# recmo/mpc-iris-code

Measured on AMD Instinct MI355X. Metric: template comparisons/sec (query×rotations×DB) + % HBM roofline, 1/2/4/8 GPU, higher is better.
Workload: dtype fp4 e2m1 MFMA -> f32 (0/+-1 products)

## Files before the change

mpc-iris-code_amd/csrc/iris_mfma.hip:

```cpp
#include <hip/hip_runtime.h>
#include <stdlib.h>

#include "iris_device.hpp"

namespace iris {

typedef int v8i __attribute__((ext_vector_type(8)));
typedef float v16f __attribute__((ext_vector_type(16)));

constexpr int kTileRecs = 32;
constexpr int kTileUint4 = kPlaneGroups * 64;
constexpr int kMfmaTiles = 4;
constexpr int kMfmaWgs = 2;
constexpr int kSplitStages = 6;
constexpr int kSplitT = 2;

__device__ __forceinline__ v16f mfma_fp4(const v8i &a, const v8i &b, const v16f &c) {
    return __builtin_amdgcn_mfma_scale_f32_32x32x64_f8f6f4(a, b, c, 4, 4, 0, 127, 0, 127);
}

struct QFrag {
    v8i am, ae;
};
__device__ __forceinline__ QFrag qfrag_of(const uint4 &qe) {
    QFrag f;
    f.ae = v8i{(int)qe.x, (int)qe.y, (int)qe.z, (int)qe.w, 0, 0, 0, 0};
    f.am = v8i{(int)(qe.x & 0x22222222u), (int)((qe.y & 0x22222222u) << 1), (int)(qe.z & 0x22222222u),
               (int)((qe.w & 0x22222222u) << 1), 0, 0, 0, 0};
    return f;
}

__device__ __forceinline__ void chunk_step(uint32_t x0, uint32_t x1, const QFrag &q, v16f &den, v16f &s) {
    const v8i bm = {(int)(x0 & 0x22222222u), (int)(x0 & 0x11111111u), (int)(x1 & 0x22222222u),
                    (int)(x1 & 0x11111111u), 0, 0, 0, 0};
    const v8i be = {(int)(x0 & 0xAAAAAAAAu), (int)((x0 << 1) & 0xAAAAAAAAu), (int)(x1 & 0xAAAAAAAAu),
                    (int)((x1 << 1) & 0xAAAAAAAAu), 0, 0, 0, 0};
    den = mfma_fp4(q.am, bm, den);
    s = mfma_fp4(q.ae, be, s);
}

typedef unsigned int u32x4 __attribute__((ext_vector_type(4)));
__device__ __forceinline__ uint4 stream_load(const uint4 *p) {
    const u32x4 v = __builtin_nontemporal_load((const u32x4 *)p);
    return make_uint4(v.x, v.y, v.z, v.w);
}

enum { MF_COUNTS = 0, MF_SEARCH = 1, MF_MATCH = 2, MF_TOPK = 3 };

template <int MODE, int T = kMfmaTiles, int KS = 1, bool FUSED = false>
__global__ void __launch_bounds__(64 * kWaveSlots, kMfmaWgs)
    template_mfma_kernel(const uint4 *__restrict__ db, const uint4 *__restrict__ qfrag, uint64_t tile0,
                         uint64_t ntiles, uint64_t first, uint64_t end, uint16_t *__restrict__ num_out,
                         uint16_t *__restrict__ den_out, double *__restrict__ dist_out,
                         Partial *__restrict__ partials, FusedFinish fin, MatchSink ms) {
    constexpr int W = kWaveSlots;
    static_assert(KS == 1 || (W % KS == 0 && kPlaneGroups % KS == 0), "K-split geometry");
    const int lane = threadIdx.x & 63;
    const int wslot = threadIdx.x >> 6;
    const int slice = wslot % KS;
    const uint64_t wave = (uint64_t)blockIdx.x * (W / KS) + wslot / KS;
    const uint64_t tw = wave * T;
    const bool active = tw < ntiles;
    constexpr int kG = kPlaneGroups / KS;
    const int g0 = slice * kG;

    v16f den[T], s[T];
#pragma unroll
    for (int t = 0; t < T; ++t) {
#pragma unroll
        for (int i = 0; i < 16; ++i) {
            den[t][i] = 0.f;
            s[t][i] = 0.f;
        }
    }

    if (active) {
        const uint4 *dp[T];
#pragma unroll
        for (int t = 0; t < T; ++t) {
            const uint64_t rel = (tw + t < ntiles) ? tw + t : ntiles - 1;
            dp[t] = db + (tile0 + rel) * (uint64_t)kTileUint4 + lane;
        }
        const uint4 *qp = qfrag + lane;
        struct Stage {
            uint4 d[T];
            uint4 q0, q1;
        };
        auto load = [&](Stage &st, int g) {
            g = (g < kG ? g : kG - 1) + g0;
#pragma unroll
            for (int t = 0; t < T; ++t) st.d[t] = stream_load(dp[t] + g * 64);
            st.q0 = qp[(2 * g) * 64];
            st.q1 = qp[(2 * g + 1) * 64];
            __builtin_amdgcn_sched_barrier(0);
        };
        auto compute = [&](const Stage &st) {
            const QFrag f0 = qfrag_of(st.q0);
#pragma unroll
            for (int t = 0; t < T; ++t) chunk_step(st.d[t].x, st.d[t].y, f0, den[t], s[t]);
            const QFrag f1 = qfrag_of(st.q1);
#pragma unroll
            for (int t = 0; t < T; ++t) chunk_step(st.d[t].z, st.d[t].w, f1, den[t], s[t]);
        };
        if constexpr (KS > 1) {
            Stage st[kSplitStages];
#pragma unroll
            for (int i = 0; i < kSplitStages - 1; ++i) load(st[i], i);
#pragma unroll
            for (int g = 0; g < kG; ++g) {
                if (g + kSplitStages - 1 < kG) load(st[(g + kSplitStages - 1) % kSplitStages], g + kSplitStages - 1);
                compute(st[g % kSplitStages]);
            }
        } else {
            Stage sa, sb, sc;
            load(sa, 0);
            load(sb, 1);
            int g = 0;
#pragma unroll 1
            for (; g + 3 <= kG; g += 3) {
                load(sc, g + 2);
                compute(sa);
                load(sa, g + 3);
                compute(sb);
                load(sb, g + 4);
                compute(sc);
            }
            if constexpr (kG % 3 >= 1) compute(sa);
            if constexpr (kG % 3 == 2) compute(sb);
        }
    }
    if constexpr (KS > 1) {
        __shared__ float red[W][T][32][64];
        if (slice != 0) {
#pragma unroll
            for (int t = 0; t < T; ++t)
#pragma unroll
                for (int i = 0; i < 16; ++i) {
                    red[wslot][t][i][lane] = den[t][i];
                    red[wslot][t][16 + i][lane] = s[t][i];
                }
        }
        __syncthreads();
        if (slice == 0) {
#pragma unroll
            for (int k = 1; k < KS; ++k)
#pragma unroll
                for (int t = 0; t < T; ++t)
#pragma unroll
                    for (int i = 0; i < 16; ++i) {
                        den[t][i] += red[wslot + k][t][i][lane];
                        s[t][i] += red[wslot + k][t][16 + i][lane];
                    }
        }
    }

    const int h = lane >> 5;
    Partial best = partial_none();
    bool hit[T];
    uint32_t hn[T], hd[T];
    int hr[T];
    uint64_t hi[T];
    uint64_t twe = tw, wave_e = wave;
    if constexpr (MODE == MF_TOPK) {
        uint32_t tx = threadIdx.x;
        asm volatile("" : "+v"(tx));
        wave_e = (uint64_t)blockIdx.x * (W / KS) + (tx >> 6) / KS;
        twe = wave_e * T;
    }
#pragma unroll
    for (int t = 0; t < T; ++t) {
        const uint64_t t0 = (tile0 + twe + t) * kTileRecs;
        const bool tv = active && (twe + t < ntiles) && slice == 0;
        if constexpr (MODE == MF_COUNTS) {
            __shared__ __attribute__((aligned(16))) uint16_t sh_out[W][1024];
            uint16_t *lds = sh_out[wslot];
            if (num_out)
                store_tile_rows(num_out, lds, t0, first, end, tv, lane,
                                [&](int r) { return (uint16_t)(((int)den[t][r] - (int)s[t][r]) >> 1); });
            if (den_out)
                store_tile_rows(den_out, lds, t0, first, end, tv, lane,
                                [&](int r) { return (uint16_t)(uint32_t)den[t][r]; });
        } else {
            const uint64_t tg = t0 + (lane & 31);
            const bool valid = tv && tg >= first && tg < end;
            const uint64_t o = tg - first;
            uint32_t bn, bd;
            int br;
            best_rotation(lane, [&](int r, uint32_t &nn, uint32_t &dd) {
                dd = (uint32_t)den[t][r];
                nn = (uint32_t)(((int)dd - (int)s[t][r]) >> 1);
            }, bn, bd, br);
            if constexpr (MODE == MF_MATCH) {
                hit[t] = match_hit(ms, valid && h == 0, bn, bd);
                hn[t] = bn;
                hd[t] = bd;
                hr[t] = br;
                hi[t] = o;
                continue;
            }
            if constexpr (MODE == MF_TOPK) {
                hn[t] = bn;
                hd[t] = valid && h == 0 ? bd : 0;
                hr[t] = br;
                continue;
            }
            if (valid && dist_out && h == 0) dist_out[o] = bd ? (double)bn / (double)bd : __builtin_inf();
            Partial c;
            c.num = bn;
            c.den = valid ? bd : 0;
            c.rot = br;
            c.pad = 0;
            c.idx = o;
            if (partial_better_dev(c, best)) best = c;
        }
    }
    if constexpr (MODE == MF_MATCH) append_matches<T>(ms, lane, hit, hn, hd, hr, hi);
    if constexpr (MODE == MF_TOPK) {
#pragma unroll
        for (int t = 0; t < T; ++t) {
            Partial c;
            c.num = hn[t];
            c.den = hd[t];
            c.rot = hr[t];
            c.pad = 0;
            c.idx = (tile0 + twe + t) * kTileRecs + (lane & 31) - first;
            topk_insert(best, (uint32_t)ms.cap, lane, c, true);
        }
        if (slice == 0) topk_store(ms, wave_e, lane, best);
    }
    if constexpr (MODE == MF_SEARCH) {
#pragma unroll
        for (int off = 32; off >= 1; off >>= 1) {
            const Partial ot = partial_shfl_xor(best, off);
            if (partial_better_dev(ot, best)) best = ot;
        }
        __shared__ Partial sh[W];
        if (lane == 0) sh[wslot] = best;
        __syncthreads();
        Partial b = sh[0];
        if (threadIdx.x == 0) {
#pragma unroll
            for (int w = 1; w < W; ++w)
                if (partial_better_dev(sh[w], b)) b = sh[w];
            if constexpr (!FUSED) partials[blockIdx.x] = b;
        }
        if constexpr (FUSED) fold_partials_last(partials, b, fin);
    }
}


struct QueryFrags {
    const uint4 *q[4];
};

template <int NQ>
__global__ void __launch_bounds__(256, 2)
    template_multi_kernel(const uint4 *__restrict__ db, QueryFrags qf, uint64_t tile0, uint64_t ntiles,
                          uint64_t first, uint64_t end, Partial *__restrict__ partials) {
    constexpr int T = 4 / NQ;
    const int lane = threadIdx.x & 63;
    const int wslot = threadIdx.x >> 6;
    const uint64_t wave = (uint64_t)blockIdx.x * kWaveSlots + wslot;
    const uint64_t tw = wave * T;
    const bool active = tw < ntiles;

    v16f den[NQ][T], s[NQ][T];
#pragma unroll
    for (int qi = 0; qi < NQ; ++qi)
#pragma unroll
        for (int t = 0; t < T; ++t)
#pragma unroll
            for (int i = 0; i < 16; ++i) {
                den[qi][t][i] = 0.f;
                s[qi][t][i] = 0.f;
            }

    if (active) {
        const uint4 *dp[T];
#pragma unroll
        for (int t = 0; t < T; ++t) {
            const uint64_t rel = (tw + t < ntiles) ? tw + t : ntiles - 1;
            dp[t] = db + (tile0 + rel) * (uint64_t)kTileUint4 + lane;
        }
        struct Stage {
            uint4 d[T];
            uint4 q[NQ][2];
        };
        auto load = [&](Stage &st, int g) {
            g = g < kPlaneGroups ? g : kPlaneGroups - 1;
#pragma unroll
            for (int t = 0; t < T; ++t) st.d[t] = stream_load(dp[t] + g * 64);
#pragma unroll
            for (int qi = 0; qi < NQ; ++qi) {
                st.q[qi][0] = qf.q[qi][(2 * g) * 64 + lane];
                st.q[qi][1] = qf.q[qi][(2 * g + 1) * 64 + lane];
            }
            __builtin_amdgcn_sched_barrier(0);
        };
        auto compute = [&](const Stage &st) {
#pragma unroll
            for (int qi = 0; qi < NQ; ++qi) {
                const QFrag f0 = qfrag_of(st.q[qi][0]);
#pragma unroll
                for (int t = 0; t < T; ++t) chunk_step(st.d[t].x, st.d[t].y, f0, den[qi][t], s[qi][t]);
                const QFrag f1 = qfrag_of(st.q[qi][1]);
#pragma unroll
                for (int t = 0; t < T; ++t) chunk_step(st.d[t].z, st.d[t].w, f1, den[qi][t], s[qi][t]);
            }
        };
        Stage sa, sb, sc;
        load(sa, 0);
        load(sb, 1);
        int g = 0;
#pragma unroll 1
        for (; g + 3 <= kPlaneGroups; g += 3) {
            load(sc, g + 2);
            compute(sa);
            load(sa, g + 3);
            compute(sb);
            load(sb, g + 4);
            compute(sc);
        }
        if (g < kPlaneGroups) compute(sa);
    }

    Partial best[NQ];
#pragma unroll
    for (int qi = 0; qi < NQ; ++qi) best[qi] = partial_none();
#pragma unroll
    for (int t = 0; t < T; ++t) {
        const uint64_t tg = (tile0 + tw + t) * kTileRecs + (lane & 31);
        const bool valid = active && (tw + t < ntiles) && tg >= first && tg < end;
#pragma unroll
        for (int qi = 0; qi < NQ; ++qi) {
            uint32_t bn, bd;
            int br;
            best_rotation(lane, [&](int r, uint32_t &nn, uint32_t &dd) {
                dd = (uint32_t)den[qi][t][r];
                nn = (uint32_t)(((int)dd - (int)s[qi][t][r]) >> 1);
            }, bn, bd, br);
            Partial c;
            c.num = bn;
            c.den = valid ? bd : 0;
            c.rot = br;
            c.pad = 0;
            c.idx = tg - first;
            if (partial_better_dev(c, best[qi])) best[qi] = c;
        }
    }
    __shared__ Partial sh[NQ][kWaveSlots];
#pragma unroll
    for (int qi = 0; qi < NQ; ++qi) {
#pragma unroll
        for (int off = 32; off >= 1; off >>= 1) {
            const Partial ot = partial_shfl_xor(best[qi], off);
            if (partial_better_dev(ot, best[qi])) best[qi] = ot;
        }
        if (lane == 0) sh[qi][wslot] = best[qi];
    }
    __syncthreads();
    if (threadIdx.x < NQ) {
        const int qi = threadIdx.x;
        Partial b = sh[qi][0];
#pragma unroll
        for (int w = 1; w < kWaveSlots; ++w)
            if (partial_better_dev(sh[qi][w], b)) b = sh[qi][w];
        partials[(uint64_t)qi * gridDim.x + blockIdx.x] = b;
    }
}


typedef const __attribute__((address_space(1))) u32x4 *GlobalFrag;
__device__ __forceinline__ uint4 frag_load(GlobalFrag p) {
    const u32x4 v = *p;
    return make_uint4(v.x, v.y, v.z, v.w);
}

template <int NQ, int T>
__device__ __forceinline__ void share_round(const uint4 *__restrict__ db, const GlobalFrag (&qf)[NQ], uint64_t tile0,
                                            uint64_t ntiles, uint64_t tw, uint64_t first, uint64_t end, int lane,
                                            Partial (&best)[NQ]) {
    const bool active = tw < ntiles;
    v16f den[NQ][T], s[NQ][T];
#pragma unroll
    for (int qi = 0; qi < NQ; ++qi)
#pragma unroll
        for (int t = 0; t < T; ++t)
#pragma unroll
            for (int i = 0; i < 16; ++i) {
                den[qi][t][i] = 0.f;
                s[qi][t][i] = 0.f;
            }

    if (active) {
        const uint4 *dp[T];
#pragma unroll
        for (int t = 0; t < T; ++t) {
            const uint64_t rel = (tw + t < ntiles) ? tw + t : ntiles - 1;
            dp[t] = db + (tile0 + rel) * (uint64_t)kTileUint4 + lane;
        }
        struct Stage {
            uint4 d[T];
            uint4 q[NQ][2];
        };
        auto load = [&](Stage &st, int g) {
            g = g < kPlaneGroups ? g : kPlaneGroups - 1;
#pragma unroll
            for (int t = 0; t < T; ++t) st.d[t] = stream_load(dp[t] + g * 64);
#pragma unroll
            for (int qi = 0; qi < NQ; ++qi) {
                st.q[qi][0] = frag_load(qf[qi] + (2 * g) * 64 + lane);
                st.q[qi][1] = frag_load(qf[qi] + (2 * g + 1) * 64 + lane);
            }
            __builtin_amdgcn_sched_barrier(0);
        };
        auto compute = [&](const Stage &st) {
#pragma unroll
            for (int qi = 0; qi < NQ; ++qi) {
                const QFrag f0 = qfrag_of(st.q[qi][0]);
#pragma unroll
                for (int t = 0; t < T; ++t) chunk_step(st.d[t].x, st.d[t].y, f0, den[qi][t], s[qi][t]);
                const QFrag f1 = qfrag_of(st.q[qi][1]);
#pragma unroll
                for (int t = 0; t < T; ++t) chunk_step(st.d[t].z, st.d[t].w, f1, den[qi][t], s[qi][t]);
            }
        };
        Stage sa, sb, sc;
        load(sa, 0);
        load(sb, 1);
        int g = 0;
#pragma unroll 1
        for (; g + 3 <= kPlaneGroups; g += 3) {
            load(sc, g + 2);
            compute(sa);
            load(sa, g + 3);
            compute(sb);
            load(sb, g + 4);
            compute(sc);
        }
        if constexpr (kPlaneGroups % 3 >= 1) compute(sa);
        if constexpr (kPlaneGroups % 3 == 2) compute(sb);
    }

#pragma unroll
    for (int t = 0; t < T; ++t) {
        const uint64_t tg = (tile0 + tw + t) * kTileRecs + (lane & 31);
        const bool valid = active && (tw + t < ntiles) && tg >= first && tg < end;
#pragma unroll
        for (int qi = 0; qi < NQ; ++qi) {
            uint32_t bn, bd;
            int br;
            best_rotation(lane, [&](int r, uint32_t &nn, uint32_t &dd) {
                dd = (uint32_t)den[qi][t][r];
                nn = (uint32_t)(((int)dd - (int)s[qi][t][r]) >> 1);
            }, bn, bd, br);
            Partial c;
            c.num = bn;
            c.den = valid ? bd : 0;
            c.rot = br;
            c.pad = 0;
            c.idx = tg - first;
            if (partial_better_dev(c, best[qi])) best[qi] = c;
        }
    }
}

template <int NQ, int N>
__device__ __forceinline__ void share_stash(Partial (&best)[NQ], int lane, int pos, Partial *sh) {
#pragma unroll
    for (int qi = 0; qi < NQ; ++qi) {
#pragma unroll
        for (int off = 32; off >= 1; off >>= 1) {
            const Partial ot = partial_shfl_xor(best[qi], off);
            if (partial_better_dev(ot, best[qi])) best[qi] = ot;
        }
        if (lane == 0) sh[qi * N + pos] = best[qi];
    }
}

typedef __attribute__((address_space(1))) Partial *GlobalPartial;
template <int NQ, int N>
__device__ __forceinline__ void share_finish(const Partial *sh, const GlobalPartial (&out)[NQ]) {
    __syncthreads();
    if (threadIdx.x < NQ) {
        const int qi = threadIdx.x;
        Partial b = sh[qi * N];
#pragma unroll
        for (int w = 1; w < N; ++w)
            if (partial_better_dev(sh[qi * N + w], b)) b = sh[qi * N + w];
        const GlobalPartial o = out[qi] + blockIdx.x;
        o->num = b.num;
        o->den = b.den;
        o->rot = b.rot;
        o->pad = b.pad;
        o->idx = b.idx;
    }
}

__global__ void __launch_bounds__(64 * kWaveSlots, kMfmaWgs)
    template_share_kernel(const uint4 *__restrict__ db, const uint4 *__restrict__ qfrag, uint64_t tile0, uint64_t ntiles,
                          uint64_t first, uint64_t end, Partial *__restrict__ partials, const GuestSlot *slot,
                          const uint32_t *own_done, unsigned long long *count, uint32_t even_only) {
    __shared__ uint32_t sh_flag[2];
    __shared__ uint64_t sh_guest[3];
    if (threadIdx.x == 0) {
        const uint32_t dn =
            own_done ? __hip_atomic_load(own_done + blockIdx.x, __ATOMIC_RELAXED, __HIP_MEMORY_SCOPE_AGENT) : 0u;
        uint32_t rdy = 0;
        if (slot && !dn && !(even_only && (blockIdx.x & 1)))
            rdy = __hip_atomic_load(&slot->ready, __ATOMIC_RELAXED, __HIP_MEMORY_SCOPE_AGENT);
        if (rdy) {
            __builtin_amdgcn_fence(__ATOMIC_ACQUIRE, "agent");
            sh_guest[0] = (uint64_t)slot->frag;
            sh_guest[1] = (uint64_t)slot->partials;
            sh_guest[2] = (uint64_t)slot->done;
        }
        sh_flag[0] = dn;
        sh_flag[1] = rdy;
    }
    __syncthreads();
    if (__builtin_amdgcn_readfirstlane(sh_flag[0])) return;
    const bool shared = __builtin_amdgcn_readfirstlane(sh_flag[1]) != 0;
    const int lane = threadIdx.x & 63;
    const int wslot = __builtin_amdgcn_readfirstlane(threadIdx.x >> 6);
    const uint64_t tw = ((uint64_t)blockIdx.x * kWaveSlots + wslot) * kMfmaTiles;
    auto uniform64 = [](uint64_t v) {
        const uint32_t lo = (uint32_t)__builtin_amdgcn_readfirstlane((int)(uint32_t)v);
        const uint32_t hi = (uint32_t)__builtin_amdgcn_readfirstlane((int)(uint32_t)(v >> 32));
        return (uint64_t)hi << 32 | lo;
    };
    constexpr int kRounds = kMfmaTiles / 2;
    __shared__ Partial sh_best[2 * kRounds * kWaveSlots];
    if (!shared) {
        Partial best[1] = {partial_none()};
        const GlobalFrag qf[1] = {(GlobalFrag)qfrag};
        share_round<1, kMfmaTiles>(db, qf, tile0, ntiles, tw, first, end, lane, best);
        share_stash<1, kWaveSlots>(best, lane, wslot, sh_best);
        const GlobalPartial out[1] = {(GlobalPartial)partials};
        share_finish<1, kWaveSlots>(sh_best, out);
        return;
    }
    const GlobalFrag qf[2] = {(GlobalFrag)qfrag, (GlobalFrag)uniform64(sh_guest[0])};
#pragma unroll
    for (int rd = 0; rd < kRounds; ++rd) {
        Partial best[2] = {partial_none(), partial_none()};
        share_round<2, 2>(db, qf, tile0, ntiles, tw + 2 * rd, first, end, lane, best);
        share_stash<2, kRounds * kWaveSlots>(best, lane, rd * kWaveSlots + wslot, sh_best);
    }
    const GlobalPartial out[2] = {(GlobalPartial)partials, (GlobalPartial)uniform64(sh_guest[1])};
    __attribute__((address_space(1))) uint32_t *const guest_done =
        (__attribute__((address_space(1))) uint32_t *)uniform64(sh_guest[2]);
    share_finish<2, kRounds * kWaveSlots>(sh_best, out);
    if (threadIdx.x == 1) {
        __hip_atomic_store(guest_done + blockIdx.x, 1u, __ATOMIC_RELAXED, __HIP_MEMORY_SCOPE_AGENT);
        if (count) atomicAdd(count, 1ull);
    }
}

__global__ void share_prepare_kernel(GuestSlot *slot, uint32_t *done, uint32_t n) {
    const uint32_t i = blockIdx.x * blockDim.x + threadIdx.x;
    if (i == 0) *slot = GuestSlot{};
    if (done && i < n) done[i] = 0;
}

__global__ void share_publish_kernel(GuestSlot *slot, const void *frag, Partial *partials, uint32_t *done) {
    slot->frag = frag;
    slot->partials = partials;
    slot->done = done;
    __hip_atomic_store(&slot->ready, 1u, __ATOMIC_RELEASE, __HIP_MEMORY_SCOPE_AGENT);
}

__global__ void share_delay_kernel(uint64_t ticks) {
    const uint64_t t0 = wall_clock64();
    while (wall_clock64() - t0 < ticks) __builtin_amdgcn_s_sleep(8);
}


__global__ void __launch_bounds__(256) pack_tiles_kernel(const uint32_t *__restrict__ staging,
                                                         uint4 *__restrict__ db, uint64_t t_first, uint64_t n) {
    const uint64_t total = n * (uint64_t)(2 * kPlaneGroups);
    for (uint64_t tid = (uint64_t)blockIdx.x * blockDim.x + threadIdx.x; tid < total;
         tid += (uint64_t)gridDim.x * blockDim.x) {
        const uint64_t i = tid % n, gh = tid / n;
        const int g = (int)(gh >> 1), h = (int)(gh & 1);
        const uint32_t *rec = staging + i * (2 * kPlaneDwords);
        const int w0 = 4 * g + h, w1 = 4 * g + 2 + h;
        const uint32_t em0 = rec[kPlaneDwords + w0], ep0 = rec[w0], em1 = rec[kPlaneDwords + w1], ep1 = rec[w1];
        const uint64_t t = t_first + i;
        uint4 v;
        v.x = xpack(em0 & 0xFFFFu, ep0 & 0xFFFFu);
        v.y = xpack(em0 >> 16, ep0 >> 16);
        v.z = xpack(em1 & 0xFFFFu, ep1 & 0xFFFFu);
        v.w = xpack(em1 >> 16, ep1 >> 16);
        db[(t / kTileRecs) * (uint64_t)kTileUint4 + (uint64_t)g * 64 + (t % kTileRecs) + 32 * h] = v;
    }
}

__global__ void __launch_bounds__(256) unpack_tiles_kernel(const uint4 *__restrict__ db, uint32_t *__restrict__ staging,
                                                           uint64_t t_first, uint64_t n) {
    const uint64_t total = n * (uint64_t)(2 * kPlaneGroups);
    for (uint64_t tid = (uint64_t)blockIdx.x * blockDim.x + threadIdx.x; tid < total;
         tid += (uint64_t)gridDim.x * blockDim.x) {
        const uint64_t i = tid % n, gh = tid / n;
        const int g = (int)(gh >> 1), h = (int)(gh & 1);
        const uint64_t t = t_first + i;
        const uint4 v = db[(t / kTileRecs) * (uint64_t)kTileUint4 + (uint64_t)g * 64 + (t % kTileRecs) + 32 * h];
        uint32_t a, b, c, d;
        xunpack(v.x, a, b);
        xunpack(v.y, c, d);
        uint32_t *rec = staging + i * (2 * kPlaneDwords);
        const int w0 = 4 * g + h, w1 = 4 * g + 2 + h;
        rec[kPlaneDwords + w0] = a | (c << 16);
        rec[w0] = b | (d << 16);
        xunpack(v.z, a, b);
        xunpack(v.w, c, d);
        rec[kPlaneDwords + w1] = a | (c << 16);
        rec[w1] = b | (d << 16);
    }
}

__global__ void __launch_bounds__(256) generate_tiles_kernel(uint4 *__restrict__ db, uint64_t t_first, uint64_t n,
                                                             uint64_t key, uint64_t global_index0) {
    const uint64_t total = n * (uint64_t)(2 * kPlaneGroups);
    for (uint64_t tid = (uint64_t)blockIdx.x * blockDim.x + threadIdx.x; tid < total;
         tid += (uint64_t)gridDim.x * blockDim.x) {
        const uint64_t i = tid % n, gh = tid / n;
        const int g = (int)(gh >> 1), h = (int)(gh & 1);
        const uint64_t gt = global_index0 + i;
        const uint64_t m0 = gen_limb(key, gt * 400 + 200 + 2 * g), m1 = gen_limb(key, gt * 400 + 200 + 2 * g + 1);
        const uint64_t p0 = gen_limb(key, gt * 400 + 2 * g), p1 = gen_limb(key, gt * 400 + 2 * g + 1);
        const uint32_t em0 = (uint32_t)(m0 >> (32 * h)), ep0 = (uint32_t)(p0 >> (32 * h));
        const uint32_t em1 = (uint32_t)(m1 >> (32 * h)), ep1 = (uint32_t)(p1 >> (32 * h));
        const uint64_t t = t_first + i;
        uint4 v;
        v.x = xpack(em0 & 0xFFFFu, ep0 & 0xFFFFu);
        v.y = xpack(em0 >> 16, ep0 >> 16);
        v.z = xpack(em1 & 0xFFFFu, ep1 & 0xFFFFu);
        v.w = xpack(em1 >> 16, ep1 >> 16);
        db[(t / kTileRecs) * (uint64_t)kTileUint4 + (uint64_t)g * 64 + (t % kTileRecs) + 32 * h] = v;
    }
}

static int tiles_grid(uint64_t total) {
    uint64_t b = (total + 255) / 256;
    if (b > 256ull * 64) b = 256ull * 64;
    return (int)(b ? b : 1);
}

int launch_pack_tiles(void *stream, const void *staging, void *db, uint64_t t_first, uint64_t n) {
    if (n == 0) return 0;
    hipLaunchKernelGGL(pack_tiles_kernel, dim3(tiles_grid(n * 2 * kPlaneGroups)), dim3(256), 0, (hipStream_t)stream,
                       (const uint32_t *)staging, (uint4 *)db, t_first, n);
    return hipGetLastError() == hipSuccess ? 0 : -1;
}

int launch_unpack_tiles(void *stream, const void *db, void *staging, uint64_t t_first, uint64_t n) {
    if (n == 0) return 0;
    hipLaunchKernelGGL(unpack_tiles_kernel, dim3(tiles_grid(n * 2 * kPlaneGroups)), dim3(256), 0, (hipStream_t)stream,
                       (const uint4 *)db, (uint32_t *)staging, t_first, n);
    return hipGetLastError() == hipSuccess ? 0 : -1;
}

int launch_generate_tiles(void *stream, void *db, uint64_t t_first, uint64_t n, uint64_t seed, uint64_t global_index0) {
    if (n == 0) return 0;
    hipLaunchKernelGGL(generate_tiles_kernel, dim3(tiles_grid(n * 2 * kPlaneGroups)), dim3(256), 0,
                       (hipStream_t)stream, (uint4 *)db, t_first, n, gen_key(seed, 0), global_index0);
    return hipGetLastError() == hipSuccess ? 0 : -1;
}

struct TileRange {
    uint64_t tile0, ntiles, grid;
    bool fusable = false;
    int tiles_per_wave;
    int ksplit;
};

constexpr uint64_t kSmallTiles = 4 * kWaveSlots * 256 * 2;
constexpr uint64_t kSplitTiles = 1024;

static TileRange tile_range(const Hooks &h, LaunchRange r) {
    TileRange t;
    t.tile0 = r.first / kTileRecs;
    const uint64_t tile1 = (r.first + r.n + kTileRecs - 1) / kTileRecs;
    t.ntiles = tile1 - t.tile0;
    t.tiles_per_wave = t.ntiles < kSmallTiles ? 1 : kMfmaTiles;
    t.ksplit = t.ntiles <= kSplitTiles ? 4 : 1;
    if (h.tiles_per_wave) {
        t.tiles_per_wave = h.tiles_per_wave == 1 ? 1 : kMfmaTiles;
        t.ksplit = 1;
    }
    if (t.ksplit > 1) {
        t.tiles_per_wave = kSplitT;
        t.grid = (t.ntiles + kSplitT - 1) / kSplitT;
        return t;
    }
    const uint64_t waves = (t.ntiles + t.tiles_per_wave - 1) / t.tiles_per_wave;
    t.grid = (waves + kWaveSlots - 1) / kWaveSlots;
    return t;
}

static TileRange search_range(const Hooks &h, LaunchRange r) {
    TileRange t = tile_range(h, r);
    t.fusable = t.grid <= (uint64_t)kFusedReduceMax;
    return t;
}

uint32_t mfma_search_partials(const Hooks &h, LaunchRange r) { return (uint32_t)search_range(h, r).grid; }

uint32_t multi_search_partials(LaunchRange r, int nq) {
    const uint64_t tile0 = r.first / kTileRecs, tile1 = (r.first + r.n + kTileRecs - 1) / kTileRecs;
    const uint64_t waves = (tile1 - tile0 + (4 / nq) - 1) / (4 / nq);
    return (uint32_t)((waves + kWaveSlots - 1) / kWaveSlots);
}

int launch_template_multi_search(void *stream, const void *db, const void *const *qfrags, int nq, LaunchRange r,
                                 Partial *partials, uint32_t *n_partials) {
    *n_partials = multi_search_partials(r, nq);
    if (r.n == 0) return 0;
    if (nq != 2) return -1;
    const uint64_t tile0 = r.first / kTileRecs, tile1 = (r.first + r.n + kTileRecs - 1) / kTileRecs;
    QueryFrags qf{};
    for (int i = 0; i < nq; ++i) qf.q[i] = (const uint4 *)qfrags[i];
    hipLaunchKernelGGL(template_multi_kernel<2>, dim3(*n_partials), dim3(256), 0, (hipStream_t)stream,
                       (const uint4 *)db, qf, tile0, tile1 - tile0, r.first, r.first + r.n, partials);
    return hipGetLastError() == hipSuccess ? 0 : -1;
}

int launch_template_mfma_counts(const Hooks &h, void *stream, const void *db, const void *qfrag, LaunchRange r, uint16_t *num_out,
                                uint16_t *den_out) {
    if (r.n == 0) return 0;
    const TileRange t = tile_range(h, r);
    auto kern = t.ksplit > 1 ? template_mfma_kernel<MF_COUNTS, kSplitT, 4>
                : t.tiles_per_wave == 1 ? template_mfma_kernel<MF_COUNTS, 1> : template_mfma_kernel<MF_COUNTS>;
    hipLaunchKernelGGL(kern, dim3((uint32_t)t.grid), dim3(256), 0, (hipStream_t)stream,
                       (const uint4 *)db, (const uint4 *)qfrag, t.tile0, t.ntiles, r.first, r.first + r.n, num_out,
                       den_out, (double *)nullptr, (Partial *)nullptr, FusedFinish{}, MatchSink{});
    return hipGetLastError() == hipSuccess ? 0 : -1;
}

int launch_template_mfma_search(const Hooks &h, void *stream, const void *db, const void *qfrag, LaunchRange r, double *dist_out,
                                Partial *partials, uint32_t *n_partials, const FusedFinish *fin) {
    const TileRange t = search_range(h, r);
    *n_partials = (uint32_t)t.grid;
    if (r.n == 0) return 0;
    const bool fused = fin && t.fusable;
    if (fin && !fused) return -1;
    auto kern = fused ? (t.ksplit > 1 ? template_mfma_kernel<MF_SEARCH, kSplitT, 4, true>
                         : t.tiles_per_wave == 1 ? template_mfma_kernel<MF_SEARCH, 1, 1, true>
                                                 : template_mfma_kernel<MF_SEARCH, kMfmaTiles, 1, true>)
                      : (t.ksplit > 1 ? template_mfma_kernel<MF_SEARCH, kSplitT, 4>
                         : t.tiles_per_wave == 1 ? template_mfma_kernel<MF_SEARCH, 1> : template_mfma_kernel<MF_SEARCH>);
    hipLaunchKernelGGL(kern, dim3((uint32_t)t.grid), dim3(64 * kWaveSlots), 0, (hipStream_t)stream,
                       (const uint4 *)db, (const uint4 *)qfrag, t.tile0, t.ntiles, r.first, r.first + r.n,
                       (uint16_t *)nullptr, (uint16_t *)nullptr, dist_out, partials, fin ? *fin : FusedFinish{},
                       MatchSink{});
    return hipGetLastError() == hipSuccess ? 0 : -1;
}

bool share_search_ok(const Hooks &h, LaunchRange r) {
    if (r.n == 0 || fused_search_ok(h, r)) return false;
    const TileRange t = search_range(h, r);
    return t.ksplit == 1 && t.tiles_per_wave == kMfmaTiles;
}

int launch_template_share_search(const Hooks &h, void *stream, const void *db, const void *qfrag, LaunchRange r,
                                 Partial *partials, uint32_t *n_partials, const GuestSlot *slot,
                                 const uint32_t *own_done, unsigned long long *count) {
    if (!share_search_ok(h, r)) return -1;
    const TileRange t = search_range(h, r);
    *n_partials = (uint32_t)t.grid;
    const bool even_only = h.search_share_even && !own_done;
    hipLaunchKernelGGL(template_share_kernel, dim3((uint32_t)t.grid), dim3(64 * kWaveSlots), 0, (hipStream_t)stream,
                       (const uint4 *)db, (const uint4 *)qfrag, t.tile0, t.ntiles, r.first, r.first + r.n, partials,
                       slot, own_done, count, (uint32_t)even_only);
    return hipGetLastError() == hipSuccess ? 0 : -1;
}

int launch_share_prepare(void *stream, GuestSlot *slot, uint32_t *done, uint32_t n) {
    const uint32_t words = done ? (n ? n : 1) : 1;
    hipLaunchKernelGGL(share_prepare_kernel, dim3((words + 255) / 256), dim3(256), 0, (hipStream_t)stream, slot, done, n);
    return hipGetLastError() == hipSuccess ? 0 : -1;
}

int launch_share_publish(void *stream, GuestSlot *slot, const void *frag, Partial *partials, uint32_t *done) {
    hipLaunchKernelGGL(share_publish_kernel, dim3(1), dim3(1), 0, (hipStream_t)stream, slot, frag, partials, done);
    return hipGetLastError() == hipSuccess ? 0 : -1;
}

int launch_share_delay(void *stream, uint64_t ticks) {
    hipLaunchKernelGGL(share_delay_kernel, dim3(1), dim3(1), 0, (hipStream_t)stream, ticks);
    return hipGetLastError() == hipSuccess ? 0 : -1;
}

int launch_template_mfma_match(const Hooks &h, void *stream, const void *db, const void *qfrag, LaunchRange r,
                               const MatchSink &ms) {
    if (r.n == 0) return 0;
    const TileRange t = tile_range(h, r);
    auto kern = t.ksplit > 1 ? template_mfma_kernel<MF_MATCH, kSplitT, 4>
                : t.tiles_per_wave == 1 ? template_mfma_kernel<MF_MATCH, 1> : template_mfma_kernel<MF_MATCH>;
    hipLaunchKernelGGL(kern, dim3((uint32_t)t.grid), dim3(64 * kWaveSlots), 0, (hipStream_t)stream,
                       (const uint4 *)db, (const uint4 *)qfrag, t.tile0, t.ntiles, r.first, r.first + r.n,
                       (uint16_t *)nullptr, (uint16_t *)nullptr, (double *)nullptr, (Partial *)nullptr, FusedFinish{}, ms);
    return hipGetLastError() == hipSuccess ? 0 : -1;
}

uint64_t mfma_topk_units(const Hooks &h, LaunchRange r) {
    const TileRange t = tile_range(h, r);
    return t.grid * (uint64_t)(t.ksplit > 1 ? 1 : kWaveSlots);
}

int launch_template_mfma_topk(const Hooks &h, void *stream, const void *db, const void *qfrag, LaunchRange r,
                              const MatchSink &ts) {
    if (r.n == 0) return 0;
    const TileRange t = tile_range(h, r);
    auto kern = t.ksplit > 1 ? template_mfma_kernel<MF_TOPK, kSplitT, 4>
                : t.tiles_per_wave == 1 ? template_mfma_kernel<MF_TOPK, 1> : template_mfma_kernel<MF_TOPK>;
    hipLaunchKernelGGL(kern, dim3((uint32_t)t.grid), dim3(64 * kWaveSlots), 0, (hipStream_t)stream,
                       (const uint4 *)db, (const uint4 *)qfrag, t.tile0, t.ntiles, r.first, r.first + r.n,
                       (uint16_t *)nullptr, (uint16_t *)nullptr, (double *)nullptr, (Partial *)nullptr, FusedFinish{}, ts);
    return hipGetLastError() == hipSuccess ? 0 : -1;
}

bool fused_search_ok(const Hooks &h, LaunchRange r) {
    if (!h.fused_reduce) return false;
    if (r.n == 0) return false;
    return search_range(h, r).fusable;
}

}
```

Measured before the change: 82.78 billion.

## Stage shared query fragments through LDS ring so each wave fetches one chunk

```diff
diff --git a/mpc-iris-code_amd/csrc/iris_mfma.hip b/mpc-iris-code_amd/csrc/iris_mfma.hip
--- a/mpc-iris-code_amd/csrc/iris_mfma.hip
+++ b/mpc-iris-code_amd/csrc/iris_mfma.hip
@@ -377,75 +377,13 @@
 }
 
 template <int NQ, int T>
-__device__ __forceinline__ void share_round(const uint4 *__restrict__ db, const GlobalFrag (&qf)[NQ], uint64_t tile0,
-                                            uint64_t ntiles, uint64_t tw, uint64_t first, uint64_t end, int lane,
-                                            Partial (&best)[NQ]) {
-    const bool active = tw < ntiles;
-    v16f den[NQ][T], s[NQ][T];
-#pragma unroll
-    for (int qi = 0; qi < NQ; ++qi)
-#pragma unroll
-        for (int t = 0; t < T; ++t)
-#pragma unroll
-            for (int i = 0; i < 16; ++i) {
-                den[qi][t][i] = 0.f;
-                s[qi][t][i] = 0.f;
-            }
-
-    if (active) {
-        const uint4 *dp[T];
-#pragma unroll
-        for (int t = 0; t < T; ++t) {
-            const uint64_t rel = (tw + t < ntiles) ? tw + t : ntiles - 1;
-            dp[t] = db + (tile0 + rel) * (uint64_t)kTileUint4 + lane;
-        }
-        struct Stage {
-            uint4 d[T];
-            uint4 q[NQ][2];
-        };
-        auto load = [&](Stage &st, int g) {
-            g = g < kPlaneGroups ? g : kPlaneGroups - 1;
-#pragma unroll
-            for (int t = 0; t < T; ++t) st.d[t] = stream_load(dp[t] + g * 64);
-#pragma unroll
-            for (int qi = 0; qi < NQ; ++qi) {
-                st.q[qi][0] = frag_load(qf[qi] + (2 * g) * 64 + lane);
-                st.q[qi][1] = frag_load(qf[qi] + (2 * g + 1) * 64 + lane);
-            }
-            __builtin_amdgcn_sched_barrier(0);
-        };
-        auto compute = [&](const Stage &st) {
-#pragma unroll
-            for (int qi = 0; qi < NQ; ++qi) {
-                const QFrag f0 = qfrag_of(st.q[qi][0]);
-#pragma unroll
-                for (int t = 0; t < T; ++t) chunk_step(st.d[t].x, st.d[t].y, f0, den[qi][t], s[qi][t]);
-                const QFrag f1 = qfrag_of(st.q[qi][1]);
-#pragma unroll
-                for (int t = 0; t < T; ++t) chunk_step(st.d[t].z, st.d[t].w, f1, den[qi][t], s[qi][t]);
-            }
-        };
-        Stage sa, sb, sc;
-        load(sa, 0);
-        load(sb, 1);
-        int g = 0;
-#pragma unroll 1
-        for (; g + 3 <= kPlaneGroups; g += 3) {
-            load(sc, g + 2);
-            compute(sa);
-            load(sa, g + 3);
-            compute(sb);
-            load(sb, g + 4);
-            compute(sc);
-        }
-        if constexpr (kPlaneGroups % 3 >= 1) compute(sa);
-        if constexpr (kPlaneGroups % 3 == 2) compute(sb);
-    }
-
+__device__ __forceinline__ void round_candidates(const v16f (&den)[NQ][T], const v16f (&s)[NQ][T], uint64_t tile0,
+                                                 uint64_t ntiles, uint64_t tw, uint64_t first, uint64_t end, int lane,
+                                                 Partial (&best)[NQ]) {
 #pragma unroll
     for (int t = 0; t < T; ++t) {
         const uint64_t tg = (tile0 + tw + t) * kTileRecs + (lane & 31);
-        const bool valid = active && (tw + t < ntiles) && tg >= first && tg < end;
+        const bool valid = (tw + t < ntiles) && tg >= first && tg < end;
 #pragma unroll
         for (int qi = 0; qi < NQ; ++qi) {
             uint32_t bn, bd;
@@ -463,6 +401,157 @@
             if (partial_better_dev(c, best[qi])) best[qi] = c;
         }
     }
+}
+
+template <int NQ, int T>
+__device__ __forceinline__ void share_round(const uint4 *__restrict__ db, const GlobalFrag (&qf)[NQ], uint64_t tile0,
+                                            uint64_t ntiles, uint64_t tw, uint64_t first, uint64_t end, int lane,
+                                            Partial (&best)[NQ]) {
+    const bool active = tw < ntiles;
+    v16f den[NQ][T], s[NQ][T];
+#pragma unroll
+    for (int qi = 0; qi < NQ; ++qi)
+#pragma unroll
+        for (int t = 0; t < T; ++t)
+#pragma unroll
+            for (int i = 0; i < 16; ++i) {
+                den[qi][t][i] = 0.f;
+                s[qi][t][i] = 0.f;
+            }
+
+    if (active) {
+        const uint4 *dp[T];
+#pragma unroll
+        for (int t = 0; t < T; ++t) {
+            const uint64_t rel = (tw + t < ntiles) ? tw + t : ntiles - 1;
+            dp[t] = db + (tile0 + rel) * (uint64_t)kTileUint4 + lane;
+        }
+        struct Stage {
+            uint4 d[T];
+            uint4 q[NQ][2];
+        };
+        auto load = [&](Stage &st, int g) {
+            g = g < kPlaneGroups ? g : kPlaneGroups - 1;
+#pragma unroll
+            for (int t = 0; t < T; ++t) st.d[t] = stream_load(dp[t] + g * 64);
+#pragma unroll
+            for (int qi = 0; qi < NQ; ++qi) {
+                st.q[qi][0] = frag_load(qf[qi] + (2 * g) * 64 + lane);
+                st.q[qi][1] = frag_load(qf[qi] + (2 * g + 1) * 64 + lane);
+            }
+            __builtin_amdgcn_sched_barrier(0);
+        };
+        auto compute = [&](const Stage &st) {
+#pragma unroll
+            for (int qi = 0; qi < NQ; ++qi) {
+                const QFrag f0 = qfrag_of(st.q[qi][0]);
+#pragma unroll
+                for (int t = 0; t < T; ++t) chunk_step(st.d[t].x, st.d[t].y, f0, den[qi][t], s[qi][t]);
+                const QFrag f1 = qfrag_of(st.q[qi][1]);
+#pragma unroll
+                for (int t = 0; t < T; ++t) chunk_step(st.d[t].z, st.d[t].w, f1, den[qi][t], s[qi][t]);
+            }
+        };
+        Stage sa, sb, sc;
+        load(sa, 0);
+        load(sb, 1);
+        int g = 0;
+#pragma unroll 1
+        for (; g + 3 <= kPlaneGroups; g += 3) {
+            load(sc, g + 2);
+            compute(sa);
+            load(sa, g + 3);
+            compute(sb);
+            load(sb, g + 4);
+            compute(sc);
+        }
+        if constexpr (kPlaneGroups % 3 >= 1) compute(sa);
+        if constexpr (kPlaneGroups % 3 == 2) compute(sb);
+    }
+    round_candidates<NQ, T>(den, s, tile0, ntiles, tw, first, end, lane, best);
+}
+
+constexpr int kStagedDepth = 4;
+typedef uint4 FragRing[2][2][2][2][64];
+
+template <int DEPTH>
+__device__ __forceinline__ void staged_round(const uint4 *__restrict__ db, const GlobalFrag (&qf)[2], uint64_t tile0,
+                                             uint64_t ntiles, uint64_t tw, uint64_t first, uint64_t end, int lane,
+                                             int wslot, FragRing &ring, Partial (&best)[2]) {
+    constexpr int T = 2;
+    static_assert(kWaveSlots == 4 && DEPTH >= 3, "one fetch per wave: 2 queries x 2 chunks of a step");
+    v16f den[2][T], s[2][T];
+#pragma unroll
+    for (int qi = 0; qi < 2; ++qi)
+#pragma unroll
+        for (int t = 0; t < T; ++t)
+#pragma unroll
+            for (int i = 0; i < 16; ++i) {
+                den[qi][t][i] = 0.f;
+                s[qi][t][i] = 0.f;
+            }
+
+    const uint4 *dp[T];
+#pragma unroll
+    for (int t = 0; t < T; ++t) {
+        const uint64_t rel = (tw + t < ntiles) ? tw + t : ntiles - 1;
+        dp[t] = db + (tile0 + rel) * (uint64_t)kTileUint4 + lane;
+    }
+    const int fq = wslot >> 1, fc = wslot & 1;
+    const GlobalFrag fp = (fq ? qf[1] : qf[0]) + fc * 64 + lane;
+    struct Stage {
+        uint4 d[T];
+        uint4 f;
+    };
+    auto load = [&](Stage &st, int g) {
+        g = g < kPlaneGroups ? g : kPlaneGroups - 1;
+#pragma unroll
+        for (int t = 0; t < T; ++t) st.d[t] = stream_load(dp[t] + g * 64);
+        st.f = frag_load(fp + (2 * g) * 64);
+        __builtin_amdgcn_sched_barrier(0);
+    };
+    auto stage_frag = [&](const Stage &st, int slot) {
+        const QFrag f = qfrag_of(st.f);
+        ring[slot][fq][fc][0][lane] = make_uint4(f.am[0], f.am[1], f.am[2], f.am[3]);
+        ring[slot][fq][fc][1][lane] = st.f;
+    };
+    auto operand = [&](int slot, int qi, int c, int e) {
+        const uint4 v = ring[slot][qi][c][e][lane];
+        return v8i{(int)v.x, (int)v.y, (int)v.z, (int)v.w, 0, 0, 0, 0};
+    };
+    auto compute = [&](const Stage &st, int slot) {
+#pragma unroll
+        for (int c = 0; c < 2; ++c)
+#pragma unroll
+            for (int qi = 0; qi < 2; ++qi) {
+                QFrag f;
+                f.am = operand(slot, qi, c, 0);
+                f.ae = operand(slot, qi, c, 1);
+#pragma unroll
+                for (int t = 0; t < T; ++t)
+                    chunk_step(c ? st.d[t].z : st.d[t].x, c ? st.d[t].w : st.d[t].y, f, den[qi][t], s[qi][t]);
+            }
+    };
+    auto step = [&](Stage &free_, const Stage &cur, const Stage &next, int g) {
+        load(free_, g + DEPTH - 1);
+        compute(cur, g & 1);
+        stage_frag(next, (g + 1) & 1);
+        __syncthreads();
+    };
+    Stage st[DEPTH];
+#pragma unroll
+    for (int i = 0; i < DEPTH - 1; ++i) load(st[i], i);
+    stage_frag(st[0], 0);
+    __syncthreads();
+    int g = 0;
+#pragma unroll 1
+    for (; g + DEPTH <= kPlaneGroups; g += DEPTH) {
+#pragma unroll
+        for (int i = 0; i < DEPTH; ++i) step(st[(i + DEPTH - 1) % DEPTH], st[i], st[(i + 1) % DEPTH], g + i);
+    }
+#pragma unroll
+    for (int i = 0; i < kPlaneGroups % DEPTH; ++i) step(st[(i + DEPTH - 1) % DEPTH], st[i], st[(i + 1) % DEPTH], g + i);
+    round_candidates<2, T>(den, s, tile0, ntiles, tw, first, end, lane, best);
 }
 
 template <int NQ, int N>
@@ -531,6 +620,7 @@
     };
     constexpr int kRounds = kMfmaTiles / 2;
     __shared__ Partial sh_best[2 * kRounds * kWaveSlots];
+    __shared__ FragRing sh_ring;
     if (!shared) {
         Partial best[1] = {partial_none()};
         const GlobalFrag qf[1] = {(GlobalFrag)qfrag};
@@ -544,7 +634,7 @@
 #pragma unroll
     for (int rd = 0; rd < kRounds; ++rd) {
         Partial best[2] = {partial_none(), partial_none()};
-        share_round<2, 2>(db, qf, tile0, ntiles, tw + 2 * rd, first, end, lane, best);
+        staged_round<kStagedDepth>(db, qf, tile0, ntiles, tw + 2 * rd, first, end, lane, wslot, sh_ring, best);
         share_stash<2, kRounds * kWaveSlots>(best, lane, rd * kWaveSlots + wslot, sh_best);
     }
     const GlobalPartial out[2] = {(GlobalPartial)partials, (GlobalPartial)uniform64(sh_guest[1])};
```

Result: faster. 84.44 billion (median of 6 runs) (+2.0%).
